# johannes-graeter/limo

Measured on NVIDIA H100. Metric: BA windows/s (30 KF, 3k LM, 40k obs), higher is better.
Workload: dtype f64

## Files before the change

limo_b200/csrc/kba_api.cu:

```cuda
#include <algorithm>
#include <atomic>
#include <chrono>
#include <cmath>
#include <cstdio>
#include <cstdlib>
#include <cstring>
#include <memory>
#include <string>
#include <thread>
#include <vector>

#include <cuda_runtime.h>

#include "kba_b200.h"
#include "kba_kernels.h"

using namespace kba;

static thread_local std::string g_last_error;
static int fail(int code, const std::string& msg) {
    g_last_error = msg;
    return code;
}
#define CU(call)                                                                                              \
// ... 713 lines not shown
        ws.free_rows = window_rows(w[i]);
        ws.n_chunks = d.n_chunks; ws.n_groups = d.n_groups; ws.n_lm = w[i].n_lm;
        d.nr_cap = nr_cap_of(ws.rows);
        d.plane_reg_weight = w[i].plane_reg_weight; d.plane_dist_fixed = w[i].plane_dist_fixed;
        d.s_off = soff;
        soff += (long long)d.nr_cap * d.nr_cap;
        kf += w[i].n_kf; cam += w[i].n_cam; lm += w[i].n_lm; obs += w[i].n_obs; chunks += d.n_chunks; gp += w[i].n_gp;
        bd.max_obs = std::max(bd.max_obs, w[i].n_obs); bd.max_lm = std::max(bd.max_lm, w[i].n_lm);
        bd.max_kf = std::max(bd.max_kf, w[i].n_kf); bd.max_gp = std::max(bd.max_gp, w[i].n_gp);
    }
    b->lc.knobs = read_knobs();
    b->lc.plan = make_plan(shapes.data(), n_windows, h->sm_count, b->lc.knobs, purpose);
    apply_plan(b);
    const int nr_cap_max = b->lc.plan.nr_cap_max;
    if (obs > 2000000000LL) { b->release(); delete b; return fail(KBA_ERR_CAPACITY, "batch exceeds 2^31 observations"); }
    if (nr_cap_max > kMaxReducedRows) {
        b->release();
        delete b;
        return fail(KBA_ERR_CAPACITY, "reduced system larger than 640 rows (106 keyframes, or 63 with ground-plane blocks)");
    }
    bd.tot_kf = kf; bd.tot_cam = cam; bd.tot_lm = lm; bd.tot_obs = obs; bd.tot_chunks = (int)chunks; bd.tot_gp = gp;
    bd.tot_groups = (int)groups;
    b->lc.sm_count = h->sm_count;
    bd.cost_parts = std::max((bd.max_obs + 255) / 256, (bd.max_obs / 16 + bd.max_lm / 32 + 4 + 7) / 8);
    bd.bs_parts = (bd.max_lm + 15) / 16;
    const bool hp = !b->lc.plan.device_pack;
    int bad = 0;
    bad |= b->desc.alloc(n_windows, true);
    bad |= b->pose0.alloc(7 * kf, true); bad |= b->plane0.alloc(4 * kf, true); bad |= b->kf_fixed.alloc(kf, true);
    bad |= b->cam.alloc(kCamStride * cam, true);
    bad |= b->lm0.alloc(3 * lm, hp); bad |= b->lm_weight.alloc(lm, hp); bad |= b->lm_ptr.alloc(lm + n_windows, hp);
    bad |= b->obs_kf.alloc(obs, hp); bad |= b->obs_cam.alloc(obs, hp); bad |= b->obs_lm.alloc(obs, hp);
    bad |= b->obs_u.alloc(obs, hp); bad |= b->obs_v.alloc(obs, hp); bad |= b->obs_d.alloc(obs, hp);
    bad |= b->kf_ptr.alloc(kf + n_windows, hp); bad |= b->pm_lm.alloc(obs, hp); bad |= b->pm_cam.alloc(obs, hp);
    bad |= b->pm_u.alloc(obs, hp); bad |= b->pm_v.alloc(obs, hp); bad |= b->pm_d.alloc(obs, hp);
    bad |= b->chunk_lm0.alloc(chunks, hp); bad |= b->chunk_lm1.alloc(chunks, hp);
    bad |= b->chunk_k0.alloc(chunks, hp); bad |= b->chunk_k1.alloc(chunks, hp);
    bad |= b->lm_orig.alloc(lm, hp); bad |= b->obs_rank.alloc(obs, hp);
    if (hp) bad |= b->obs_orig.alloc(obs, true);
    bad |= b->grp_k0.alloc(groups, hp); bad |= b->grp_k1.alloc(groups, hp);
    if (b->lc.plan.device_pack) {
        bad |= b->r_lm_ptr.alloc(lm + n_windows, true); bad |= b->r_obs_kf.alloc(obs, true); bad |= b->r_obs_cam.alloc(obs, true);
        bad |= b->r_obs_u.alloc(obs, true); bad |= b->r_obs_v.alloc(obs, true); bad |= b->r_obs_d.alloc(obs, true);
        bad |= b->r_lm_pos.alloc(3 * lm, true); bad |= b->r_lm_weight.alloc(lm, true); bad |= b->r_gp_lm.alloc(gp, true);
        bad |= b->lm_user.alloc(3 * lm, true); bad |= b->rej_user.alloc(lm, true);
        bad |= b->dev_alloc(&b->raw.lm_inv, lm);
    }
    bad |= b->dev_alloc(&bd.grp_t0, groups); bad |= b->dev_alloc(&bd.grp_t1, groups); bad |= b->dev_alloc(&bd.grp_rs, groups);
    bad |= b->dev_alloc(&bd.grp_tiles, groups);
    bad |= b->dev_alloc(&bd.lin_tile, (size_t)(obs / 16) + (size_t)(lm / 32) + 4 * (size_t)n_windows + 4);
#ifdef KBA_PROF
    bad |= b->dev_alloc(&bd.prof, 16);
    if (!bad) cudaMemset(bd.prof, 0, 16 * sizeof(unsigned long long));
#endif
    bad |= b->dev_alloc(&bd.rt[0], (size_t)kPoseStride * kf); bad |= b->dev_alloc(&bd.rt[1], (size_t)kPoseStride * kf);
    {
        bd.panel_cap = 0;
        bd.vpanel = nullptr;
        bad |= b->dev_alloc(&bd.chunk_poff, chunks); bad |= b->dev_alloc(&bd.chunk_rs, chunks);
    }
    bad |= b->dev_alloc(&bd.chunk_t0, chunks); bad |= b->dev_alloc(&bd.chunk_t1, chunks); bad |= b->dev_alloc(&bd.obs_row, obs);
    bad |= b->state.alloc(n_windows, true); bad |= b->log.alloc((size_t)n_windows * kIterLogCap, true);
    for (int q = 0; q < 2; ++q) { bad |= b->pose_out[q].alloc(7 * kf, true); bad |= b->lm_out[q].alloc(3 * lm, hp); }
    bad |= b->lm_active.alloc(lm, hp); bad |= b->n_active.alloc(1, true); bad |= b->jac_obs.alloc(1, true);
    bad |= b->plane_out[0].alloc(4 * kf, true); bad |= b->plane_out[1].alloc(4 * kf, true);
    bad |= b->gp_lm.alloc(gp, hp); bad |= b->gp_kf.alloc(gp, true); bad |= b->gp_weight.alloc(gp, true); bad |= b->gp_of_lm.alloc(lm, hp); bad |= b->gp_shared.alloc(gp, hp);
    bad |= b->dev_alloc(&bd.gp_lin, 14 * gp); bad |= b->dev_alloc(&bd.vgp, 30 * gp);
    bad |= b->dev_alloc(&bd.gp_kfb, gp ? 65 * (size_t)kf : 0);
    bad |= b->dev_alloc(&bd.gp_cost_x, n_windows); bad |= b->dev_alloc(&bd.gp_cost_c, n_windows);
    bad |= b->dev_alloc(&bd.off_pose, kf); bad |= b->dev_alloc(&bd.off_dir, kf); bad |= b->dev_alloc(&bd.off_dist, kf);
    bad |= b->dev_alloc(&bd.bkf, 27 * kf);
    bad |= b->dev_alloc(&bd.scale_f, (size_t)n_windows * nr_cap_max); bad |= b->dev_alloc(&bd.lambda_f, (size_t)n_windows * nr_cap_max);
    bad |= b->dev_alloc(&bd.grad_f, (size_t)n_windows * nr_cap_max); bad |= b->dev_alloc(&bd.delta_f, (size_t)n_windows * nr_cap_max);
    bad |= b->dev_alloc(&bd.lm_scale, 3 * lm); bad |= b->dev_alloc(&bd.lm_linv, 6 * lm); bad |= b->dev_alloc(&bd.lm_z, 3 * lm);
    bad |= b->dev_alloc(&bd.lm_g, 3 * lm); bad |= b->dev_alloc(&bd.lm_lambda, 3 * lm); bad |= b->dev_alloc(&bd.trim_val, 3 * lm);
    bad |= b->dev_alloc(&bd.trim_reject, lm);
    bad |= b->dev_alloc(&bd.res, 3 * obs); bad |= b->dev_alloc(&bd.jp, 18 * obs);
    if (!bd.fused) bad |= b->dev_alloc(&bd.jl, 9 * obs);
    else { bad |= b->dev_alloc(&bd.vobs, 18 * obs); bad |= b->dev_alloc(&bd.lm_run, lm); }
    bad |= b->dev_alloc(&bd.cost_part_x, (size_t)n_windows * bd.cost_parts); bad |= b->dev_alloc(&bd.cost_part_c, (size_t)n_windows * bd.cost_parts);
    bad |= b->dev_alloc(&bd.bs_part, (size_t)n_windows * bd.bs_parts * 4);
    bad |= b->dev_alloc(&bd.sred, (size_t)soff * bd.p_split); bad |= b->dev_alloc(&bd.amat, (size_t)soff);
    bad |= b->dev_alloc(&bd.chol_w, (size_t)n_windows * 32 * 32); bad |= b->dev_alloc(&bd.chol_invd, (size_t)n_windows * nr_cap_max);
    if (bad) {
        const std::string msg = std::string("device/pinned allocation failed: ") + cudaGetErrorString(cudaGetLastError());
        b->release(); delete b;
        return fail(KBA_ERR_CUDA, msg);
    }
    bd.desc = b->desc.d; bd.state = b->state.d; bd.log = b->log.d;
    bd.pose0 = b->pose0.d; bd.plane0 = b->plane0.d; bd.pose[0] = b->pose_out[0].d; bd.pose[1] = b->pose_out[1].d;
    bd.kf_fixed = b->kf_fixed.d; bd.cam = b->cam.d;
    bd.lm0 = b->lm0.d; bd.lm[0] = b->lm_out[0].d; bd.lm[1] = b->lm_out[1].d; bd.lm_weight = b->lm_weight.d;
    bd.lm_active = b->lm_active.d; bd.lm_ptr = b->lm_ptr.d;
    bd.obs_kf = b->obs_kf.d; bd.obs_cam = b->obs_cam.d; bd.obs_lm = b->obs_lm.d;
// ... 2106 lines not shown
```

limo_b200/csrc/kba_device.cuh:

```cuda
#pragma once
#include <cstdint>
#include <cuda_runtime.h>

#include "kba_plan.h"

namespace kba {

constexpr int kMaxKf = 128;
constexpr int kMaxCam = 8;
constexpr int kPoseStride = 12;
constexpr int kCamStride = 16;
constexpr int kIterLogCap = 160;

struct WinDesc {
    int n_kf, n_cam, n_lm, n_obs, n_gp;
    int kf_off, cam_off, lm_off, obs_off, gp_off;
    int chunk_off, n_chunks;
    int grp_off, n_groups;
    int scale_kf0, scale_kf1;
    double scale_weight, scale_value;
    double plane_reg_weight;
    int plane_dist_fixed, landmarks_fixed;
    int speed_kf;
    int idle;
// ... 42 lines not shown
    double radius, decrease_factor;
    double x_cost, x_norm, gmax;
    double f_model, f_step_sq, f_xnorm_sq, f_gmax;
    unsigned long long t_solve_start;
    SolveSummary solves[8];
};

struct BatchDev {
    int n_win;
    int max_obs, max_lm, max_kf, max_gp;
    long long tot_obs, tot_lm, tot_kf, tot_cam, tot_gp;
    WinDesc* desc;
    WinState* state;
    IterRecord* log;
    double* pose0;
    double* plane0;
    double* pose[2];
    double* rt[2];
    double* plane[2];
    uint8_t* kf_fixed;
    int* off_pose;
    int* off_dir;
    int* off_dist;
    double* bkf;
    double* scale_f;
    double* cam;
    double* lm0;
    double* lm[2];
    double* lm_weight;
    uint8_t* lm_active;
    uint8_t* lm_active0;
    int* lm_ptr;
    double* lm_scale;
    double* lm_linv;
    double* lm_z;
    double* lm_g;
    double* lm_lambda;
    double* trim_val;
    uint8_t* trim_reject;
    int* obs_kf;
    int* obs_cam;
    int* obs_lm;
    int* obs_rank;
    float* obs_u, *obs_v, *obs_d;
    int* kf_ptr;
    int* pm_lm;
    int* pm_cam;
// ... 337 lines not shown
```

limo_b200/csrc/kba_kernels.cu:

```cuda
#include "kba_device.cuh"
#include "kba_kernels.h"
#include "kba_regularisers.cuh"
#include "kba_controller.cuh"
#include "kba_prep.cuh"
#include "kba_linearize.cuh"

#include <cfloat>
#include <cstdio>
#include <cstdlib>
#include <cmath>
#include <type_traits>

namespace kba {

__global__ void __launch_bounds__(256) k_shard_planes(BatchDev bd) {
    if (bd.state[0].phase != PH_SOLVE_BEGIN) return;
    const WinDesc& wd = bd.desc[0];
    for (int k = threadIdx.x; k < wd.n_kf; k += blockDim.x) bd.kf_gp_glob[k] = 0;
    __syncthreads();
    for (int j = threadIdx.x; j < bd.lm_total; j += blockDim.x) {
        const int kp = (int)bd.gp_kf_glob[j];
        if (kp > 0 && bd.act_glob[j]) bd.kf_gp_glob[kp - 1] = 1;
    }
}
// ... 154 lines not shown
                const int t0 = bd.chunk_t0[wd.chunk_off + c], t1 = bd.chunk_t1[wd.chunk_off + c];
                int rs = 0;
                if (t1 > t0) {
                    const int rows = 8 * (t1 - t0) + ((trhs >= t0 && trhs < t1) ? 0 : 8);
                    rs = ((rows - 4 + 15) / 16) * 16 + 4;
                }
                bd.chunk_rs[wd.chunk_off + c] = rs;
                bd.chunk_poff[wd.chunk_off + c] = poff;
                poff += 96 * rs;
            }
        }
    }
}

__global__ void __launch_bounds__(256) k_panel_zero(BatchDev bd) {
    const int w = blockIdx.y;
    if (bd.fused || bd.state[w].phase != PH_SOLVE_BEGIN || bd.desc[w].landmarks_fixed) return;
    double2* p = reinterpret_cast<double2*>(bd.vpanel + bd.desc[w].panel_off);
    const long long n2 = bd.panel_cap / 2;
    for (long long i = (long long)blockIdx.x * blockDim.x + threadIdx.x; i < n2; i += (long long)gridDim.x * blockDim.x)
        p[i] = make_double2(0.0, 0.0);
}

template <bool kJac, int kMinBlocks, typename TLin, bool kJl = true>
__global__ void __launch_bounds__(256, kMinBlocks) k_eval_obs(BatchDev bd, SolveParams sp, int tiles) {
    const int w = blockIdx.y;
    WinState& st = bd.state[w];
    const WinDesc& wd = bd.desc[w];
    const int n_obs = wd.n_obs, obs_off = wd.obs_off, lm_off = wd.lm_off;
    if (st.phase != PH_ITERATE) return;
    if (kJac && !st.need_linearize) return;
    if (!kJac && st.solve_failed) return;
    __shared__ __align__(16) double s_pose[kMaxKf * kPoseStride];
    __shared__ __align__(16) double s_cam[kMaxCam * kCamStride];
    __shared__ __align__(8) uint64_t s_bar;
    __shared__ double s_red[8];
    __shared__ int s_cnt[8];
    constexpr bool kF32 = sizeof(TLin) == 4;
    __shared__ float s_pose_f[kF32 ? kMaxKf * kPoseStride : 1];
    __shared__ float s_cam_f[kF32 ? kMaxCam * kCamStride : 1];
    const int buf = kJac ? st.cur : 1 - st.cur;
    const double* __restrict__ lm_buf = bd.lm[buf];
    const int i0 = blockIdx.x * tiles * 256 + threadIdx.x;
    int idx_b = (i0 < n_obs) ? bd.obs_lm[(size_t)obs_off + i0] : -1;
    int idx_a = (tiles > 1 && i0 + 256 < n_obs) ? bd.obs_lm[(size_t)obs_off + i0 + 256] : -1;
    int L = -1, kfi = 0, cami = 0, row = -1;
    float u = 0.f, v = 0.f, d = 0.f;
    double p0 = 0, p1 = 0, p2 = 0, wgt = 0;
    unsigned char act = 0;
    if (idx_b >= 0) {
        const size_t o = (size_t)obs_off + i0;
        L = lm_off + idx_b;
        kfi = bd.obs_kf[o]; cami = bd.obs_cam[o];
        if (kJac) row = bd.obs_row[o];
        u = bd.obs_u[o]; v = bd.obs_v[o]; d = bd.obs_d[o];
        p0 = lm_buf[3 * (size_t)L]; p1 = lm_buf[3 * (size_t)L + 1]; p2 = lm_buf[3 * (size_t)L + 2];
        wgt = bd.lm_weight[L];
        act = bd.lm_active[L];
    }
    stage_window_bulk(wd, bd.rt[buf], bd.cam, s_pose, s_cam, &s_bar);
    if (kF32) {
        for (int i = threadIdx.x; i < wd.n_kf * kPoseStride; i += blockDim.x) s_pose_f[i] = (float)s_pose[i];
        for (int i = threadIdx.x; i < wd.n_cam * kCamStride; i += blockDim.x) s_cam_f[i] = (float)s_cam[i];
        __syncthreads();
    }
    double cost = 0.0;
    int done = 0;
#pragma unroll 1
    for (int t = 0; t < tiles; ++t) {
        const int i_n = i0 + (t + 1) * 256;
        int Ln = -1, kfn = 0, camn = 0, rown = -1;
        float un = 0.f, vn = 0.f, dn = 0.f;
        double q0 = 0, q1 = 0, q2 = 0, wn = 0;
        unsigned char actn = 0;
        if (idx_a >= 0) {
            const size_t o = (size_t)obs_off + i_n;
            Ln = lm_off + idx_a;
            kfn = bd.obs_kf[o]; camn = bd.obs_cam[o];
            if (kJac) rown = bd.obs_row[o];
            un = bd.obs_u[o]; vn = bd.obs_v[o]; dn = bd.obs_d[o];
            q0 = lm_buf[3 * (size_t)Ln]; q1 = lm_buf[3 * (size_t)Ln + 1]; q2 = lm_buf[3 * (size_t)Ln + 2];
            wn = bd.lm_weight[Ln];
            actn = bd.lm_active[Ln];
        }
        idx_a = (t + 2 < tiles && i_n + 256 < n_obs) ? bd.obs_lm[(size_t)obs_off + i_n + 256] : -1;
        if (L >= 0 && act) {
            const size_t o = (size_t)obs_off + i0 + t * 256;
            const int k = kfi, c = cami;
            const double p[3] = {p0, p1, p2};
            double hr = 0.0;
            bool ok;
            if (kJac && kF32) {
                double r[3], raw[2];
                ok = eval_observation<double, false>(
                    s_pose + kPoseStride * k, s_cam + kCamStride * c, p, (double)u, (double)v, (double)d, wgt,
                    sp.reprojection_thres * sp.reprojection_thres, sp.depth_thres * sp.depth_thres, r, nullptr, nullptr, hr,
                    raw);
                if (ok) {
                    const float pf[3] = {(float)p0, (float)p1, (float)p2};
                    float hrf;
                    float* resf = reinterpret_cast<float*>(bd.res) + o;
                    float* jpf = reinterpret_cast<float*>(bd.jp) + o;
                    float* jlf = reinterpret_cast<float*>(bd.jl) + o;
                    eval_observation_store<float, kJl>(
                        s_pose_f + kPoseStride * k, s_cam_f + kCamStride * c, pf, u, v, d, (float)wgt,
                        (float)(sp.reprojection_thres * sp.reprojection_thres), (float)(sp.depth_thres * sp.depth_thres),
                        resf, jpf, jlf, (size_t)bd.tot_obs, row >= 0 || !kJl, hrf);
                }
            } else if (kJac) {
                ok = eval_observation_store<double, kJl>(
                    s_pose + kPoseStride * k, s_cam + kCamStride * c, p, (double)u, (double)v, (double)d, wgt,
                    sp.reprojection_thres * sp.reprojection_thres, sp.depth_thres * sp.depth_thres, bd.res + o, bd.jp + o,
                    bd.jl + o, (size_t)bd.tot_obs, row >= 0 || !kJl, hr);
            } else {
                double r[3], raw[2];
                ok = eval_observation<double, false>(
                    s_pose + kPoseStride * k, s_cam + kCamStride * c, p, (double)u, (double)v, (double)d, wgt,
                    sp.reprojection_thres * sp.reprojection_thres, sp.depth_thres * sp.depth_thres, r, nullptr, nullptr,
                    hr, raw);
            }
            if (!ok) {
                st.eval_failed = 1;
            } else {
                cost += hr;
                ++done;
            }
        }
        L = Ln; kfi = kfn; cami = camn; row = rown; u = un; v = vn; d = dn; p0 = q0; p1 = q1; p2 = q2; wgt = wn; act = actn;
    }
    cost = warp_sum(cost);
    if (kJac) done = __reduce_add_sync(0xffffffffu, done);
    if ((threadIdx.x & 31) == 0) { s_red[threadIdx.x >> 5] = cost; s_cnt[threadIdx.x >> 5] = done; }
    __syncthreads();
    if (threadIdx.x < tiles) {
        double s = 0.0;
        if (threadIdx.x == 0)
            for (int q = 0; q < 8; ++q) s += s_red[q];
        const int slot = blockIdx.x * tiles + threadIdx.x;
        if (slot < bd.cost_parts) (kJac ? bd.cost_part_x : bd.cost_part_c)[(size_t)w * bd.cost_parts + slot] = s;
    }
    if (kJac && threadIdx.x == 0) {
        int cnt = 0;
        for (int q = 0; q < 8; ++q) cnt += s_cnt[q];
        if (cnt) atomicAdd(bd.jac_obs, (unsigned long long)cnt);
    }
}

constexpr int kEvalTiles = 8;
template <bool kJac>
static void launch_eval_obs(const BatchDev& bd, const SolveParams& sp, cudaStream_t s) {
    const dim3 g((bd.max_obs + 256 * kEvalTiles - 1) / (256 * kEvalTiles), bd.n_win);
    if (!kJac) { k_eval_obs<false, 4, double><<<g, 256, 0, s>>>(bd, sp, kEvalTiles); return; }
    if (bd.precision == 1) {
        if (bd.fused) k_eval_obs<true, 2, float, false><<<g, 256, 0, s>>>(bd, sp, kEvalTiles);
        else k_eval_obs<true, 2, float, true><<<g, 256, 0, s>>>(bd, sp, kEvalTiles);
    } else {
        if (bd.fused) k_eval_obs<true, 2, double, false><<<g, 256, 0, s>>>(bd, sp, kEvalTiles);
        else k_eval_obs<true, 2, double, true><<<g, 256, 0, s>>>(bd, sp, kEvalTiles);
    }
    LCHK("k_eval_obs");
}

template <bool kJac>
__global__ void __launch_bounds__(256) k_gp_eval(BatchDev bd, SolveParams sp) {
    const int w = blockIdx.x;
    const WinState& st = bd.state[w];
    if (st.phase != PH_ITERATE) return;
    if (kJac && !st.need_linearize) return;
    if (!kJac && st.solve_failed) return;
    const WinDesc& wd = bd.desc[w];
    if (wd.n_gp == 0) return;
    __shared__ double s_red[8];
    const int buf = kJac ? st.cur : 1 - st.cur;
    const size_t TG = (size_t)bd.tot_gp;
    double cost = 0.0;
    for (int gi = threadIdx.x; gi < wd.n_gp; gi += blockDim.x) {
        const size_t G = (size_t)wd.gp_off + gi;
        const int L = wd.lm_off + bd.gp_lm[G];
        if (!bd.lm_active[L]) continue;
        const int k = bd.gp_kf[G];
        const double* ps = bd.pose[buf] + 7 * (size_t)(wd.kf_off + k);
// ... 57 lines not shown
        const int e = lane + 32 * s;
        int a = 0, b = 0;
        if (e < 55) { while ((a + 1) * (a + 2) / 2 <= e) ++a; b = e - a * (a + 1) / 2; }
        else if (e < 65) { a = e - 55; b = -1; }
        else { a = -1; b = -1; }
        ea[s] = a; eb[s] = b;
    }
    for (int gi = 0; gi < wd.n_gp; ++gi) {
        const size_t G = (size_t)wd.gp_off + gi;
        if (bd.gp_kf[G] != k || !bd.lm_active[wd.lm_off + bd.gp_lm[G]]) continue;
#pragma unroll
        for (int s = 0; s < 3; ++s) {
            if (ea[s] < 0) continue;
            const double va = bd.gp_lin[(1 + ea[s]) * TG + G];
            const double vb = (eb[s] >= 0) ? bd.gp_lin[(1 + eb[s]) * TG + G] : bd.gp_lin[G];
            acc[s] += va * vb;
        }
    }
#pragma unroll
    for (int s = 0; s < 3; ++s)
        if (ea[s] >= 0) bd.gp_kfb[(size_t)(wd.kf_off + k) * 65 + lane + 32 * s] = acc[s];
}

__global__ void __launch_bounds__(256, 2) k_pose_hessian(BatchDev bd, SolveParams sp) {
    const int w = blockIdx.y, k = blockIdx.x;
    const WinState& st = bd.state[w];
    if (st.phase != PH_ITERATE || !st.need_linearize) return;
    const WinDesc& wd = bd.desc[w];
    if (k >= wd.n_kf || bd.off_pose[wd.kf_off + k] < 0) return;
    __shared__ double s_pose[kPoseStride];
    __shared__ double s_cam[kMaxCam * kCamStride];
    __shared__ double s_red[8][27];
    __shared__ double s_acc[9][256];
    __shared__ long long s_ob;
    __shared__ int s_lm_off, s_e1;
    if (threadIdx.x == 0) {
        s_ob = wd.obs_off; s_lm_off = wd.lm_off; s_e1 = bd.kf_ptr[wd.kf_off + w + k + 1];
        const double* p = bd.pose[st.cur] + 7 * (size_t)(wd.kf_off + k);
        double R[9];
        quat_to_rot<double>(p, R);
        for (int i = 0; i < 9; ++i) s_pose[i] = R[i];
        s_pose[9] = p[4]; s_pose[10] = p[5]; s_pose[11] = p[6];
    }
    for (int i = threadIdx.x; i < wd.n_cam * kCamStride; i += blockDim.x) s_cam[i] = bd.cam[(size_t)wd.cam_off * kCamStride + i];
    __syncthreads();
    double acc[18];
#pragma unroll
    for (int q = 0; q < 18; ++q) acc[q] = 0.0;
#pragma unroll
    for (int q = 0; q < 9; ++q) s_acc[q][threadIdx.x] = 0.0;
    const int* kp = bd.kf_ptr + wd.kf_off + w;
    const int e0 = kp[k], e1 = kp[k + 1];
    const double* __restrict__ lm_buf = bd.lm[st.cur];
    const size_t ob = (size_t)wd.obs_off;
    int e = e0 + threadIdx.x;
    int idx_b = (e < e1) ? bd.pm_lm[ob + e] : -1;
    int idx_a = (e + (int)blockDim.x < e1) ? bd.pm_lm[ob + e + blockDim.x] : -1;
    int L = -1, cam = 0;
    float u = 0.f, v = 0.f, d = 0.f;
    double p0 = 0, p1 = 0, p2 = 0, wgt = 0;
    unsigned char act = 0;
    if (idx_b >= 0) {
        L = wd.lm_off + idx_b;
        cam = bd.pm_cam[ob + e]; u = bd.pm_u[ob + e]; v = bd.pm_v[ob + e]; d = bd.pm_d[ob + e];
        p0 = lm_buf[3 * (size_t)L]; p1 = lm_buf[3 * (size_t)L + 1]; p2 = lm_buf[3 * (size_t)L + 2];
        wgt = bd.lm_weight[L]; act = bd.lm_active[L];
    }
#pragma unroll 1
    for (; e < s_e1; e += blockDim.x) {
        asm volatile("" ::: "memory");
        const size_t obs0 = (size_t)s_ob;
        const int e_end = s_e1, lm0 = s_lm_off;
        const int en = e + blockDim.x;
        int Ln = -1, camn = 0;
        float un = 0.f, vn = 0.f, dn = 0.f;
        double q0 = 0, q1 = 0, q2 = 0, wn = 0;
        unsigned char actn = 0;
        if (idx_a >= 0) {
            Ln = lm0 + idx_a;
            camn = bd.pm_cam[obs0 + en]; un = bd.pm_u[obs0 + en]; vn = bd.pm_v[obs0 + en]; dn = bd.pm_d[obs0 + en];
            q0 = lm_buf[3 * (size_t)Ln]; q1 = lm_buf[3 * (size_t)Ln + 1]; q2 = lm_buf[3 * (size_t)Ln + 2];
            wn = bd.lm_weight[Ln]; actn = bd.lm_active[Ln];
        }
        idx_a = (en + (int)blockDim.x < e_end) ? bd.pm_lm[obs0 + en + blockDim.x] : -1;
        if (act) {
            const double p[3] = {p0, p1, p2};
            double r[3], m[9], a[3], raw[2], hr;
            if (eval_factored<double, true, false>(s_pose, s_cam + kCamStride * cam, p, (double)u, (double)v, (double)d,
                                                   wgt, sp.reprojection_thres * sp.reprojection_thres,
                                                   sp.depth_thres * sp.depth_thres, r, m, a, hr, raw)) {
                double mm[6], h[3];
                gram_factored(m, mm);
#pragma unroll
                for (int c = 0; c < 3; ++c) h[c] = m[c] * r[0] + m[3 + c] * r[1] + m[6 + c] * r[2];
#pragma unroll
                for (int i = 0; i < 3; ++i) {
                    const int i1 = (i + 1) % 3, i2 = (i + 2) % 3;
                    double pr[3];
#pragma unroll
                    for (int c = 0; c < 3; ++c) pr[c] = 2.0 * (a[i1] * mm[sym3(i2, c)] - a[i2] * mm[sym3(i1, c)]);
                    const int qd = 6 * i - i * (i - 1) / 2;
#pragma unroll
                    for (int j = i; j < 3; ++j) {
                        const int j1 = (j + 1) % 3, j2 = (j + 2) % 3;
                        acc[qd + j - i] += 2.0 * (a[j1] * pr[j2] - a[j2] * pr[j1]);
                    }
#pragma unroll
                    for (int c = 0; c < 3; ++c) acc[qd + 3 - i + c] += pr[c];
                    acc[15 + i] += 2.0 * (a[i1] * h[i2] - a[i2] * h[i1]);
                }
#pragma unroll
                for (int q = 0; q < 6; ++q) s_acc[q][threadIdx.x] += mm[q];
#pragma unroll
                for (int c = 0; c < 3; ++c) s_acc[6 + c][threadIdx.x] += h[c];
            }
        }
        L = Ln; cam = camn; u = un; v = vn; d = dn; p0 = q0; p1 = q1; p2 = q2; wgt = wn; act = actn;
    }
#pragma unroll
    for (int q = 0; q < 27; ++q) {
        const double t = q < 15 ? acc[q] : q < 21 ? s_acc[q - 15][threadIdx.x] : q < 24 ? acc[q - 6] : s_acc[q - 18][threadIdx.x];
        const double v = warp_sum(t);
        if ((threadIdx.x & 31) == 0) s_red[threadIdx.x >> 5][q] = v;
    }
    __syncthreads();
    if (threadIdx.x < 27) {
        double s = 0.0;
        for (int q = 0; q < 8; ++q) s += s_red[q][threadIdx.x];
        bd.bkf[(size_t)(wd.kf_off + k) * 27 + threadIdx.x] = s;
    }
}

constexpr int kLC = 32;
constexpr int kKC = 3 * kLC;

__device__ __forceinline__ int gp_row(const BatchDev& bd, const WinDesc& wd, int k, int r) {
    if (r < 6) { const int o = bd.off_pose[wd.kf_off + k]; return o < 0 ? -1 : o + r; }
    if (r < 9) { const int o = bd.off_dir[wd.kf_off + k]; return o < 0 ? -1 : o + r - 6; }
    return bd.off_dist[wd.kf_off + k];
}

__device__ __forceinline__ void dmma(double& c0, double& c1, double a, double b) {
    asm volatile("mma.sync.aligned.m8n8k4.row.col.f64.f64.f64.f64 {%0,%1}, {%2}, {%3}, {%0,%1};\n"
                 : "+d"(c0), "+d"(c1)
                 : "d"(a), "d"(b));
}

constexpr int kGS = 64 + 4;

__global__ void __launch_bounds__(256, 2) k_schur_syrk(BatchDev bd) {
    const int w = blockIdx.z;
    const WinState& st = bd.state[w];
// ... 405 lines not shown
            int rr[8], cc[8];
#pragma unroll
            for (int u = 0; u < 8; ++u) {
                const int idx = idx0 + u * nth;
                const int r = idx / ld, c = idx - r * ld;
                const bool skip = idx >= total || (kTiled ? (c >= rows || (c >> 3) > (r >> 3)) : (c > r || c >= n + 1));
                rr[u] = skip ? -1 : r; cc[u] = c;
                double s = 0.0;
                if (!skip && !wd.landmarks_fixed && c <= r && r <= n && !(r == n && c == n))
                    for (int p = 0; p < np; ++p) s += sp0[p * pstride + (size_t)r * ld + c];
                v[u] = s;
            }
#pragma unroll
            for (int u = 0; u < 8; ++u)
                if (rr[u] >= 0) A(rr[u], cc[u]) = -v[u];
        }
    }
    __syncthreads();
    PHASE_MARK(1);
    for (int idx = tid; idx < wd.n_kf * 27; idx += nth) {
        const int k = idx / 27, q = idx - 27 * k;
        const int off = bd.off_pose[wd.kf_off + k];
        if (off < 0) continue;
        const double v = bd.bkf[(size_t)(wd.kf_off + k) * 27 + q];
        if (q < 21) {
            int a = 0, rem = q;
            while (rem >= 6 - a) { rem -= 6 - a; ++a; }
            const int b = a + rem;
            A(off + b, off + a) += v;
            if (a == b) s_fdiag[off + a] = v;
        } else {
            s_g[off + q - 21] = v;
        }
    }
    __syncthreads();
    if (wd.n_gp > 0 || bd.shard_gp) {
        for (int idx = tid; idx < wd.n_kf * 65; idx += nth) {
            const int k = idx / 65, e = idx - 65 * k;
            int a, b;
            if (e < 55) { a = 0; while ((a + 1) * (a + 2) / 2 <= e) ++a; b = e - a * (a + 1) / 2; }
            else { a = e - 55; b = -1; }
            const int ra = gp_row(bd, wd, k, a);
            if (ra < 0) continue;
            const double v = bd.gp_kfb[(size_t)(wd.kf_off + k) * 65 + e];
            if (b < 0) { s_g[ra] += v; continue; }
            const int rb = gp_row(bd, wd, k, b);
            if (rb < 0) continue;
// ... 632 lines not shown
            const double* p = bd.bs_part + (size_t)q * 4;
            a += p[0]; b += p[1]; c += p[2]; g = fmax(g, p[3]);
        }
        for (int q = lane; q < bd.cost_parts; q += 32) cc += bd.cost_part_c[q];
    }
    a = warp_sum(a); b = warp_sum(b); c = warp_sum(c); g = warp_max(g);
    cc = warp_sum(cc);
    if (lane == 0) {
        bd.xs[0] = a; bd.xs[1] = b; bd.xs[2] = c; bd.xs[3] = cc;
        bd.xs[4] = (st.phase == PH_ITERATE && st.eval_failed) ? 1.0 : 0.0;
        bd.xs[5] = (st.phase == PH_ITERATE && wd.n_gp > 0) ? bd.gp_cost_c[0] : 0.0;
        for (int r = 0; r < bd.shard_world; ++r) bd.xs[16 + r] = (r == bd.shard_rank) ? g : 0.0;
    }
}
__host__ __device__ inline long long shard_gp_doubles(int shard_gp, int n_kf) { return shard_gp ? 65LL * n_kf + 1 : 0; }
__global__ void __launch_bounds__(256) k_shard_pack(BatchDev bd) {
    const WinState& st = bd.state[0];
    const WinDesc& wd = bd.desc[0];
    const size_t n_s = (size_t)wd.nr_cap * wd.nr_cap, n_b = (size_t)wd.n_kf * 27, n_c = (size_t)bd.shard_cost_parts;
    const size_t n_g = (size_t)shard_gp_doubles(bd.shard_gp, wd.n_kf), n_kb = (size_t)wd.n_kf * 65;
    const size_t i = (size_t)blockIdx.x * blockDim.x + threadIdx.x;
    const bool on = st.phase == PH_ITERATE, gp = on && wd.n_gp > 0;
    if (i < n_s) bd.x_send[i] = on ? bd.sred[i] : 0.0;
    else if (i < n_s + n_b) bd.x_send[i] = on ? bd.bkf[i - n_s] : 0.0;
    else if (i < n_s + n_b + n_kb && n_g) bd.x_send[i] = gp ? bd.gp_kfb[i - n_s - n_b] : 0.0;
    else if (i == n_s + n_b + n_kb && n_g) bd.x_send[i] = gp ? bd.gp_cost_x[0] : 0.0;
    else if (i < n_s + n_b + n_g + n_c) {
        const size_t q = i - n_s - n_b - n_g;
        bd.x_send[i] = (on && q < (size_t)bd.cost_parts) ? bd.cost_part_x[q] : 0.0;
    }
    else if (i == n_s + n_b + n_g + n_c) bd.x_send[i] = (on && st.eval_failed) ? 1.0 : 0.0;
    else if (i == n_s + n_b + n_g + n_c + 1) bd.x_send[i] = (on && st.solve_failed) ? 1.0 : 0.0;
}
__global__ void k_shard_flags(BatchDev bd) {
    WinState& st = bd.state[0];
    if (threadIdx.x != 0 || st.phase != PH_ITERATE) return;
    const WinDesc& wd = bd.desc[0];
    const double* f = bd.x_recv + (size_t)wd.nr_cap * wd.nr_cap + (size_t)wd.n_kf * 27 + shard_gp_doubles(bd.shard_gp, wd.n_kf) +
                      bd.shard_cost_parts;
    if (f[0] > 0.0) st.eval_failed = 1;
    if (f[1] > 0.0 && !st.solve_failed) st.solve_failed = 1;
}
__global__ void __launch_bounds__(256) k_shard_trim_scatter(BatchDev bd) {
    const WinState& st = bd.state[0];
    if (st.phase != PH_TRIM) return;
    const WinDesc& wd = bd.desc[0];
    const int j = blockIdx.x * blockDim.x + threadIdx.x;
// ... 260 lines not shown
    const int B = bd.n_win;
    const dim3 g_obs((bd.max_obs + 255) / 256, B);
    const dim3 g_lm((bd.max_lm + 63) / 64, B);
    if (!bd.fused) k_panel_zero<<<dim3(64, B), 256, 0, s>>>(bd);
    LCHK("k_panel_zero");
    if (bd.sharded && bd.shard_gp) k_shard_planes<<<1, 256, 0, s>>>(bd);
    LCHK("k_shard_planes");
    k_solve_begin<<<B, kBeginThreads, 0, s>>>(bd, sp); LCHK("k_solve_begin");
    const bool timed = lc.time_jacobian && lc.ev_pool && *lc.ev_used + 2 <= lc.ev_cap;
    const bool lin1 = bd.lin1 != 0;
    if (lin1) {
        if (bd.tot_gp > 0) {
            k_gp_eval<true><<<B, 256, 0, s>>>(bd, sp);
            k_gp_blocks<<<dim3((bd.max_kf + 7) / 8, B), 256, 0, s>>>(bd);
        }
        LCHK("k_gp_eval");
        if (timed) cudaEventRecord(lc.ev_pool[(*lc.ev_used)++], s);
        const int n_units = (lin_tile_bound(bd.max_obs, bd.max_lm) + kLinWarps - 1) / kLinWarps;
        const dim3 g_lin(strided_grid(lc.knobs.lin_grid, n_units, 1, 8, B, lc.sm_count, kLinMinBlocks, 6), B);
        if ((int)g_lin.x < n_units) k_linearize<true><<<g_lin, kLinThreads, 0, s>>>(bd, sp, n_units);
        else k_linearize<false><<<g_lin, kLinThreads, 0, s>>>(bd, sp, n_units);
        LCHK("k_linearize");
        if (timed) cudaEventRecord(lc.ev_pool[(*lc.ev_used)++], s);
        k_pose_hessian<<<dim3(bd.max_kf, B), 256, 0, s>>>(bd, sp); LCHK("k_pose_hessian");
    } else {
        if (timed) cudaEventRecord(lc.ev_pool[(*lc.ev_used)++], s);
        launch_eval_obs<true>(bd, sp, s);
        if (timed) cudaEventRecord(lc.ev_pool[(*lc.ev_used)++], s);
        if (bd.tot_gp > 0) {
            k_gp_eval<true><<<B, 256, 0, s>>>(bd, sp);
            k_gp_blocks<<<dim3((bd.max_kf + 7) / 8, B), 256, 0, s>>>(bd);
        }
        LCHK("k_gp_eval");
        k_pose_hessian<<<dim3(bd.max_kf, B), 256, 0, s>>>(bd, sp); LCHK("k_pose_hessian");
    }
    if (bd.fused) {
        if (!lin1) {
            k_landmark_reduce<true><<<dim3((bd.max_lm + 15) / 16, B), 256, 0, s>>>(bd, sp); LCHK("k_landmark_reduce");
            k_obs_v2<<<g_obs, 256, 0, s>>>(bd); LCHK("k_obs_v2");
        }
        const dim3 gf(bd.p_split, B);
        if (lc.plan.fused_slots == 7) k_schur_fused<7><<<gf, 512, schur_fused_smem(), s>>>(bd);
        else k_schur_fused<6><<<gf, 512, schur_fused_smem(), s>>>(bd);
        LCHK("k_schur_fused");
    } else {
        k_landmark_reduce<false><<<dim3((bd.max_lm + 15) / 16, B), 256, 0, s>>>(bd, sp); LCHK("k_landmark_reduce");
        for (int round = 0; round <= lc.max_rank; ++round) k_obs_v<<<g_obs, 256, 0, s>>>(bd, round);
        LCHK("k_obs_v");
        if (bd.tot_gp > 0) k_gp_panel<<<dim3((bd.max_gp * 10 + 255) / 256, B), 256, 0, s>>>(bd);
        LCHK("k_gp_panel");
    }
    if (bd.fused) {
    } else if (lc.plan.small_syrk) {
        k_schur_syrk_tma<<<dim3(bd.p_split, B), 512, schur_tma_smem(), s>>>(bd); LCHK("k_schur_syrk_tma");
    } else {
        const int nb = lc.plan.nr_cap_max / 64;
        k_schur_syrk<<<dim3(nb * (nb + 1) / 2, bd.p_split, B), 256, schur_smem(), s>>>(bd); LCHK("k_schur_syrk");
    }
    const dim3 g_red((lc.plan.nr_cap_max * lc.plan.nr_cap_max + 255) / 256, B);
    BatchDev bc = bd;
    if (bd.sharded) {
        if (bd.p_split > 1) k_sred_reduce<<<g_red, 256, 0, s>>>(bd, 1);
        LCHK("k_sred_reduce");
        const LaunchCfg::WinDescHost& wh = lc.shard_win;
        const long long n_s = (long long)wh.nr_cap * wh.nr_cap, n_b = (long long)wh.n_kf * 27, n_g = shard_gp_doubles(bd.shard_gp, wh.n_kf);
        const long long n_x = n_s + n_b + n_g + bd.shard_cost_parts + 2;
        k_shard_pack<<<(unsigned)((n_x + 255) / 256), 256, 0, s>>>(bd); LCHK("k_shard_pack");
        if (int rc = lc.xchg.allreduce(lc.xchg.user, bd.x_send, bd.x_recv, n_x, 0, s)) return rc;
        k_shard_flags<<<1, 32, 0, s>>>(bd); LCHK("k_shard_flags");
        bc.sred = bd.x_recv; bc.bkf = bd.x_recv + n_s; bc.cost_part_x = bd.x_recv + n_s + n_b + n_g; bc.cost_parts = bd.shard_cost_parts;
        if (n_g) { bc.gp_kfb = bd.x_recv + n_s + n_b; bc.gp_cost_x = bd.x_recv + n_s + n_b + 65LL * wh.n_kf; }
        k_sred_reduce<<<g_red, 256, 0, s>>>(bc, 2); LCHK("k_sred_reduce");
    } else if (bd.p_split > 1) {
        k_sred_reduce<<<g_red, 256, 0, s>>>(bd, 0); LCHK("k_sred_reduce");
    }
    if (bd.solve_tiled) {
        k_reduced_solve<true><<<B, 512, solve_tiled_smem(lc.plan.nr_cap_max), s>>>(bc, sp, 0); LCHK("k_reduced_solve");
    } else if (!bd.solve_split) {
        k_reduced_solve<false><<<B, 512, solve_smem(lc.plan.nr_cap_max), s>>>(bc, sp, 0); LCHK("k_reduced_solve");
    } else {
        k_reduced_solve<false><<<B, 512, solve_smem(lc.plan.nr_cap_max), s>>>(bc, sp, 1); LCHK("k_reduced_solve");
        const int strips = (lc.plan.nr_cap_max + 7) / 8;
        for (int kb = 0; kb < lc.plan.nr_cap_max; kb += kNB) {
            k_chol_diag<<<B, 32, 0, s>>>(bc, kb); LCHK("k_chol_diag");
            k_chol_panel<<<dim3((strips + 15) / 16, B), 512, 0, s>>>(bc, kb); LCHK("k_chol_panel");
            k_chol_trail<<<dim3(bd.solve_split, B), 512, trail_smem(lc.plan.nr_cap_max), s>>>(bc, kb); LCHK("k_chol_trail");
        }
        k_reduced_solve<false><<<B, 512, solve_smem(lc.plan.nr_cap_max), s>>>(bc, sp, 2); LCHK("k_reduced_solve");
    }
    if (bd.fused) {
        const int n_units = (bd.max_lm + 15) / 16;
        const int gx = strided_grid(lc.knobs.bs_grid, n_units, 1, 3, B, lc.sm_count, 2, 8);
        if (gx < n_units) k_backsub_v<true><<<dim3(gx, B), 256, 0, s>>>(bd, n_units);
        else k_backsub_v<false><<<dim3(n_units, B), 256, 0, s>>>(bd, n_units);
    }
    else k_backsub<<<dim3((bd.max_lm + 15) / 16, B), 256, 0, s>>>(bd);
    LCHK("k_backsub");
    launch_eval_obs<false>(bd, sp, s);
    if (bd.tot_gp > 0) k_gp_eval<false><<<B, 256, 0, s>>>(bd, sp);
    LCHK("k_gp_eval");
    if (bd.sharded) {
        k_shard_scalars<<<1, 32, 0, s>>>(bd); LCHK("k_shard_scalars");
        if (int rc = lc.xchg.allreduce(lc.xchg.user, bd.xs, bd.xs, 16 + bd.shard_world, 0, s)) return rc;
    }
    k_lm_update<<<(B * 32 + 127) / 128, 128, 0, s>>>(bd, sp); LCHK("k_lm_update");
    k_trim_eval<<<g_lm, 256, 0, s>>>(bd, sp); LCHK("k_trim_eval");
    if (bd.sharded) {
        k_shard_trim_scatter<<<(bd.max_lm + 255) / 256, 256, 0, s>>>(bd); LCHK("k_shard_trim_scatter");
        if (int rc = lc.xchg.allreduce(lc.xchg.user, bd.trim_send, bd.trim_glob, 3LL * bd.lm_total, 0, s)) return rc;
    }
    k_trim_select<<<B, 512, 0, s>>>(bd, sp); LCHK("k_trim_select");
    if (cnt) {
        const int gp = bd.tot_gp > 0 ? 1 : 0;
        const int prep = lin1 ? 1 : 2 + (bd.fused ? 1 : lc.max_rank + 1 + gp);
        cnt->launches_total += gp; cnt->launches_prep += gp;
        if (bd.sharded && bd.shard_gp) cnt->launches_total += 1;
        const int split = (!bd.solve_tiled && bd.solve_split) ? 1 + 3 * ((lc.plan.nr_cap_max + kNB - 1) / kNB) : 0;
        cnt->launches_total += (bd.fused ? 0 : 1) + 1 + 1 + gp + prep + 1 + (bd.p_split > 1 ? 1 : 0) + 1 + split + 1 + 1 + gp + 1 + 2;
        cnt->launches_jacobian += 1; cnt->launches_prep += prep + gp; cnt->launches_schur += 1; cnt->launches_solve += 2;
        cnt->launches_backsub += 1; cnt->launches_cost += 1 + gp; cnt->launches_update += 1; cnt->launches_trim += 2;
    }
// ... 8 lines not shown
__global__ void __launch_bounds__(256) k_loop_cond(BatchDev bd, cudaGraphConditionalHandle handle, int* pass, int max_passes) {
    int active = 0;
    for (int w = threadIdx.x; w < bd.n_win; w += blockDim.x) active += (bd.state[w].phase != PH_DONE) ? 1 : 0;
    active = __syncthreads_count(active > 0);
    if (threadIdx.x == 0) {
        const int p = *pass + 1;
        *pass = p;
        *bd.n_active = active;
        cudaGraphSetConditional(handle, (active > 0 && p < max_passes) ? 1u : 0u);
    }
}
void launch_loop_cond(const BatchDev& bd, unsigned long long handle, int* pass, int max_passes, cudaStream_t s) {
    k_loop_cond<<<1, 256, 0, s>>>(bd, (cudaGraphConditionalHandle)handle, pass, max_passes);
}

__global__ void k_force_linearize(BatchDev bd) {
    const int w = blockIdx.x * blockDim.x + threadIdx.x;
    if (w >= bd.n_win) return;
    WinState& st = bd.state[w];
    st.phase = PH_ITERATE; st.need_linearize = 1; st.iter0 = 1; st.cur = 0; st.eval_failed = 0; st.solve_failed = 0;
}
void launch_jacobian_only(const BatchDev& bd, const SolveParams& sp, cudaStream_t s) {
    const dim3 g_obs((bd.max_obs + 255) / 256, bd.n_win);
    launch_eval_obs<true>(bd, sp, s);
}
template <typename TLin>
__global__ void k_expand_jl(BatchDev bd, double* out) {
    const WinDesc& wd = bd.desc[0];
    const int i = blockIdx.x * blockDim.x + threadIdx.x;
    if (i >= wd.n_obs) return;
    const size_t o = (size_t)wd.obs_off + i, T = (size_t)bd.tot_obs;
    const double* R = bd.rt[0] + kPoseStride * (size_t)(wd.kf_off + bd.obs_kf[o]);
    const TLin* jp = reinterpret_cast<const TLin*>(bd.jp);
    for (int r = 0; r < 3; ++r) {
        const double m0 = (double)jp[(6 * r + 3) * T + o], m1 = (double)jp[(6 * r + 4) * T + o], m2 = (double)jp[(6 * r + 5) * T + o];
        for (int c = 0; c < 3; ++c) out[(size_t)(3 * r + c) * T + o] = m0 * R[c] + m1 * R[3 + c] + m2 * R[6 + c];
    }
}
void launch_expand_jl(const BatchDev& bd, double* out, cudaStream_t s) {
    const int n = (int)bd.tot_obs;
    if (bd.precision) k_expand_jl<float><<<(n + 255) / 256, 256, 0, s>>>(bd, out);
    else k_expand_jl<double><<<(n + 255) / 256, 256, 0, s>>>(bd, out);
    LCHK("k_expand_jl");
}
void launch_force_linearize(const BatchDev& bd, cudaStream_t s) {
    k_solve_begin<<<bd.n_win, kBeginThreads, 0, s>>>(bd, SolveParams{}); LCHK("k_solve_begin");
    k_force_linearize<<<(bd.n_win + 127) / 128, 128, 0, s>>>(bd); LCHK("k_force_linearize");
// ... 4 lines not shown
```

Measured before the change: 1454.

## Fuse candidate cost evaluation into pose Hessian kernel and double-buffer bkf

Replaces the separate candidate-cost eval_obs pass after backsubstitution with a k_pose_hessian<true> launch. That launch evaluates the candidate state, accumulates cost per keyframe and also precomputes the pose Hessian blocks into a second bkf buffer. The intent is that an accepted step can reuse these blocks, so the next linearization skips k_pose_hessian unless iter0. This removes a redundant per-observation pass, at the cost of a heavier candidate kernel that builds the Hessian even for steps that get rejected. It also adds buffer-index bookkeeping across cur flips.

```diff
diff --git a/limo_b200/csrc/kba_api.cu b/limo_b200/csrc/kba_api.cu
--- a/limo_b200/csrc/kba_api.cu
+++ b/limo_b200/csrc/kba_api.cu
@@ -759,7 +759,7 @@
     bd.tot_kf = kf; bd.tot_cam = cam; bd.tot_lm = lm; bd.tot_obs = obs; bd.tot_chunks = (int)chunks; bd.tot_gp = gp;
     bd.tot_groups = (int)groups;
     b->lc.sm_count = h->sm_count;
-    bd.cost_parts = std::max((bd.max_obs + 255) / 256, (bd.max_obs / 16 + bd.max_lm / 32 + 4 + 7) / 8);
+    bd.cost_parts = std::max(std::max((bd.max_obs + 255) / 256, (bd.max_obs / 16 + bd.max_lm / 32 + 4 + 7) / 8), bd.max_kf);
     bd.bs_parts = (bd.max_lm + 15) / 16;
     const bool hp = !b->lc.plan.device_pack;
     int bad = 0;
@@ -806,7 +806,7 @@
     bad |= b->dev_alloc(&bd.gp_kfb, gp ? 65 * (size_t)kf : 0);
     bad |= b->dev_alloc(&bd.gp_cost_x, n_windows); bad |= b->dev_alloc(&bd.gp_cost_c, n_windows);
     bad |= b->dev_alloc(&bd.off_pose, kf); bad |= b->dev_alloc(&bd.off_dir, kf); bad |= b->dev_alloc(&bd.off_dist, kf);
-    bad |= b->dev_alloc(&bd.bkf, 27 * kf);
+    bad |= b->dev_alloc(&bd.bkf[0], 27 * kf); bad |= b->dev_alloc(&bd.bkf[1], 27 * kf);
     bad |= b->dev_alloc(&bd.scale_f, (size_t)n_windows * nr_cap_max); bad |= b->dev_alloc(&bd.lambda_f, (size_t)n_windows * nr_cap_max);
     bad |= b->dev_alloc(&bd.grad_f, (size_t)n_windows * nr_cap_max); bad |= b->dev_alloc(&bd.delta_f, (size_t)n_windows * nr_cap_max);
     bad |= b->dev_alloc(&bd.lm_scale, 3 * lm); bad |= b->dev_alloc(&bd.lm_linv, 6 * lm); bad |= b->dev_alloc(&bd.lm_z, 3 * lm);
diff --git a/limo_b200/csrc/kba_device.cuh b/limo_b200/csrc/kba_device.cuh
--- a/limo_b200/csrc/kba_device.cuh
+++ b/limo_b200/csrc/kba_device.cuh
@@ -88,7 +88,7 @@
     int* off_pose;
     int* off_dir;
     int* off_dist;
-    double* bkf;
+    double* bkf[2];
     double* scale_f;
     double* cam;
     double* lm0;
diff --git a/limo_b200/csrc/kba_kernels.cu b/limo_b200/csrc/kba_kernels.cu
--- a/limo_b200/csrc/kba_kernels.cu
+++ b/limo_b200/csrc/kba_kernels.cu
@@ -200,15 +200,13 @@
         p[i] = make_double2(0.0, 0.0);
 }
 
-template <bool kJac, int kMinBlocks, typename TLin, bool kJl = true>
+template <int kMinBlocks, typename TLin, bool kJl = true>
 __global__ void __launch_bounds__(256, kMinBlocks) k_eval_obs(BatchDev bd, SolveParams sp, int tiles) {
     const int w = blockIdx.y;
     WinState& st = bd.state[w];
     const WinDesc& wd = bd.desc[w];
     const int n_obs = wd.n_obs, obs_off = wd.obs_off, lm_off = wd.lm_off;
-    if (st.phase != PH_ITERATE) return;
-    if (kJac && !st.need_linearize) return;
-    if (!kJac && st.solve_failed) return;
+    if (st.phase != PH_ITERATE || !st.need_linearize) return;
     __shared__ __align__(16) double s_pose[kMaxKf * kPoseStride];
     __shared__ __align__(16) double s_cam[kMaxCam * kCamStride];
     __shared__ __align__(8) uint64_t s_bar;
@@ -217,7 +215,7 @@
     constexpr bool kF32 = sizeof(TLin) == 4;
     __shared__ float s_pose_f[kF32 ? kMaxKf * kPoseStride : 1];
     __shared__ float s_cam_f[kF32 ? kMaxCam * kCamStride : 1];
-    const int buf = kJac ? st.cur : 1 - st.cur;
+    const int buf = st.cur;
     const double* __restrict__ lm_buf = bd.lm[buf];
     const int i0 = blockIdx.x * tiles * 256 + threadIdx.x;
     int idx_b = (i0 < n_obs) ? bd.obs_lm[(size_t)obs_off + i0] : -1;
@@ -230,7 +228,7 @@
         const size_t o = (size_t)obs_off + i0;
         L = lm_off + idx_b;
         kfi = bd.obs_kf[o]; cami = bd.obs_cam[o];
-        if (kJac) row = bd.obs_row[o];
+        row = bd.obs_row[o];
         u = bd.obs_u[o]; v = bd.obs_v[o]; d = bd.obs_d[o];
         p0 = lm_buf[3 * (size_t)L]; p1 = lm_buf[3 * (size_t)L + 1]; p2 = lm_buf[3 * (size_t)L + 2];
         wgt = bd.lm_weight[L];
@@ -255,7 +253,7 @@
             const size_t o = (size_t)obs_off + i_n;
             Ln = lm_off + idx_a;
             kfn = bd.obs_kf[o]; camn = bd.obs_cam[o];
-            if (kJac) rown = bd.obs_row[o];
+            rown = bd.obs_row[o];
             un = bd.obs_u[o]; vn = bd.obs_v[o]; dn = bd.obs_d[o];
             q0 = lm_buf[3 * (size_t)Ln]; q1 = lm_buf[3 * (size_t)Ln + 1]; q2 = lm_buf[3 * (size_t)Ln + 2];
             wn = bd.lm_weight[Ln];
@@ -268,7 +266,7 @@
             const double p[3] = {p0, p1, p2};
             double hr = 0.0;
             bool ok;
-            if (kJac && kF32) {
+            if (kF32) {
                 double r[3], raw[2];
                 ok = eval_observation<double, false>(
                     s_pose + kPoseStride * k, s_cam + kCamStride * c, p, (double)u, (double)v, (double)d, wgt,
@@ -285,17 +283,11 @@
                         (float)(sp.reprojection_thres * sp.reprojection_thres), (float)(sp.depth_thres * sp.depth_thres),
                         resf, jpf, jlf, (size_t)bd.tot_obs, row >= 0 || !kJl, hrf);
                 }
-            } else if (kJac) {
+            } else {
                 ok = eval_observation_store<double, kJl>(
                     s_pose + kPoseStride * k, s_cam + kCamStride * c, p, (double)u, (double)v, (double)d, wgt,
                     sp.reprojection_thres * sp.reprojection_thres, sp.depth_thres * sp.depth_thres, bd.res + o, bd.jp + o,
                     bd.jl + o, (size_t)bd.tot_obs, row >= 0 || !kJl, hr);
-            } else {
-                double r[3], raw[2];
-                ok = eval_observation<double, false>(
-                    s_pose + kPoseStride * k, s_cam + kCamStride * c, p, (double)u, (double)v, (double)d, wgt,
-                    sp.reprojection_thres * sp.reprojection_thres, sp.depth_thres * sp.depth_thres, r, nullptr, nullptr,
-                    hr, raw);
             }
             if (!ok) {
                 st.eval_failed = 1;
@@ -307,7 +299,7 @@
         L = Ln; kfi = kfn; cami = camn; row = rown; u = un; v = vn; d = dn; p0 = q0; p1 = q1; p2 = q2; wgt = wn; act = actn;
     }
     cost = warp_sum(cost);
-    if (kJac) done = __reduce_add_sync(0xffffffffu, done);
+    done = __reduce_add_sync(0xffffffffu, done);
     if ((threadIdx.x & 31) == 0) { s_red[threadIdx.x >> 5] = cost; s_cnt[threadIdx.x >> 5] = done; }
     __syncthreads();
     if (threadIdx.x < tiles) {
@@ -315,9 +307,9 @@
         if (threadIdx.x == 0)
             for (int q = 0; q < 8; ++q) s += s_red[q];
         const int slot = blockIdx.x * tiles + threadIdx.x;
-        if (slot < bd.cost_parts) (kJac ? bd.cost_part_x : bd.cost_part_c)[(size_t)w * bd.cost_parts + slot] = s;
-    }
-    if (kJac && threadIdx.x == 0) {
+        if (slot < bd.cost_parts) bd.cost_part_x[(size_t)w * bd.cost_parts + slot] = s;
+    }
+    if (threadIdx.x == 0) {
         int cnt = 0;
         for (int q = 0; q < 8; ++q) cnt += s_cnt[q];
         if (cnt) atomicAdd(bd.jac_obs, (unsigned long long)cnt);
@@ -325,16 +317,14 @@
 }
 
 constexpr int kEvalTiles = 8;
-template <bool kJac>
 static void launch_eval_obs(const BatchDev& bd, const SolveParams& sp, cudaStream_t s) {
     const dim3 g((bd.max_obs + 256 * kEvalTiles - 1) / (256 * kEvalTiles), bd.n_win);
-    if (!kJac) { k_eval_obs<false, 4, double><<<g, 256, 0, s>>>(bd, sp, kEvalTiles); return; }
     if (bd.precision == 1) {
-        if (bd.fused) k_eval_obs<true, 2, float, false><<<g, 256, 0, s>>>(bd, sp, kEvalTiles);
-        else k_eval_obs<true, 2, float, true><<<g, 256, 0, s>>>(bd, sp, kEvalTiles);
+        if (bd.fused) k_eval_obs<2, float, false><<<g, 256, 0, s>>>(bd, sp, kEvalTiles);
+        else k_eval_obs<2, float, true><<<g, 256, 0, s>>>(bd, sp, kEvalTiles);
     } else {
-        if (bd.fused) k_eval_obs<true, 2, double, false><<<g, 256, 0, s>>>(bd, sp, kEvalTiles);
-        else k_eval_obs<true, 2, double, true><<<g, 256, 0, s>>>(bd, sp, kEvalTiles);
+        if (bd.fused) k_eval_obs<2, double, false><<<g, 256, 0, s>>>(bd, sp, kEvalTiles);
+        else k_eval_obs<2, double, true><<<g, 256, 0, s>>>(bd, sp, kEvalTiles);
     }
     LCHK("k_eval_obs");
 }
@@ -438,21 +428,28 @@
         if (ea[s] >= 0) bd.gp_kfb[(size_t)(wd.kf_off + k) * 65 + lane + 32 * s] = acc[s];
 }
 
+template <bool kCand>
 __global__ void __launch_bounds__(256, 2) k_pose_hessian(BatchDev bd, SolveParams sp) {
     const int w = blockIdx.y, k = blockIdx.x;
-    const WinState& st = bd.state[w];
-    if (st.phase != PH_ITERATE || !st.need_linearize) return;
+    WinState& st = bd.state[w];
+    if (st.phase != PH_ITERATE) return;
+    if (kCand ? st.solve_failed != 0 : !(st.need_linearize && st.iter0)) return;
     const WinDesc& wd = bd.desc[w];
-    if (k >= wd.n_kf || bd.off_pose[wd.kf_off + k] < 0) return;
+    if (kCand && k >= wd.n_kf) {
+        if (threadIdx.x == 0) bd.cost_part_c[(size_t)w * bd.cost_parts + k] = 0.0;
+        return;
+    }
+    if (k >= wd.n_kf || (!kCand && bd.off_pose[wd.kf_off + k] < 0)) return;
+    const int buf = kCand ? 1 - st.cur : st.cur;
     __shared__ double s_pose[kPoseStride];
     __shared__ double s_cam[kMaxCam * kCamStride];
-    __shared__ double s_red[8][27];
-    __shared__ double s_acc[9][256];
+    __shared__ double s_red[8][kCand ? 28 : 27];
+    __shared__ double s_acc[kCand ? 10 : 9][256];
     __shared__ long long s_ob;
     __shared__ int s_lm_off, s_e1;
     if (threadIdx.x == 0) {
         s_ob = wd.obs_off; s_lm_off = wd.lm_off; s_e1 = bd.kf_ptr[wd.kf_off + w + k + 1];
-        const double* p = bd.pose[st.cur] + 7 * (size_t)(wd.kf_off + k);
+        const double* p = bd.pose[buf] + 7 * (size_t)(wd.kf_off + k);
         double R[9];
         quat_to_rot<double>(p, R);
         for (int i = 0; i < 9; ++i) s_pose[i] = R[i];
@@ -464,10 +461,10 @@
 #pragma unroll
     for (int q = 0; q < 18; ++q) acc[q] = 0.0;
 #pragma unroll
-    for (int q = 0; q < 9; ++q) s_acc[q][threadIdx.x] = 0.0;
+    for (int q = 0; q < (kCand ? 10 : 9); ++q) s_acc[q][threadIdx.x] = 0.0;
     const int* kp = bd.kf_ptr + wd.kf_off + w;
     const int e0 = kp[k], e1 = kp[k + 1];
-    const double* __restrict__ lm_buf = bd.lm[st.cur];
+    const double* __restrict__ lm_buf = bd.lm[buf];
     const size_t ob = (size_t)wd.obs_off;
     int e = e0 + threadIdx.x;
     int idx_b = (e < e1) ? bd.pm_lm[ob + e] : -1;
@@ -502,9 +499,10 @@
         if (act) {
             const double p[3] = {p0, p1, p2};
             double r[3], m[9], a[3], raw[2], hr;
-            if (eval_factored<double, true, false>(s_pose, s_cam + kCamStride * cam, p, (double)u, (double)v, (double)d,
+            if (eval_factored<double, true, kCand>(s_pose, s_cam + kCamStride * cam, p, (double)u, (double)v, (double)d,
                                                    wgt, sp.reprojection_thres * sp.reprojection_thres,
                                                    sp.depth_thres * sp.depth_thres, r, m, a, hr, raw)) {
+                if (kCand) s_acc[9][threadIdx.x] += hr;
                 double mm[6], h[3];
                 gram_factored(m, mm);
 #pragma unroll
@@ -529,21 +527,25 @@
                 for (int q = 0; q < 6; ++q) s_acc[q][threadIdx.x] += mm[q];
 #pragma unroll
                 for (int c = 0; c < 3; ++c) s_acc[6 + c][threadIdx.x] += h[c];
+            } else if (kCand) {
+                bd.state[blockIdx.y].eval_failed = 1;
             }
         }
         L = Ln; cam = camn; u = un; v = vn; d = dn; p0 = q0; p1 = q1; p2 = q2; wgt = wn; act = actn;
     }
 #pragma unroll
-    for (int q = 0; q < 27; ++q) {
+    for (int q = 0; q < (kCand ? 28 : 27); ++q) {
         const double t = q < 15 ? acc[q] : q < 21 ? s_acc[q - 15][threadIdx.x] : q < 24 ? acc[q - 6] : s_acc[q - 18][threadIdx.x];
         const double v = warp_sum(t);
         if ((threadIdx.x & 31) == 0) s_red[threadIdx.x >> 5][q] = v;
     }
     __syncthreads();
-    if (threadIdx.x < 27) {
+    if (threadIdx.x < (kCand ? 28 : 27)) {
         double s = 0.0;
         for (int q = 0; q < 8; ++q) s += s_red[q][threadIdx.x];
-        bd.bkf[(size_t)(wd.kf_off + k) * 27 + threadIdx.x] = s;
+        const int half = kCand ? 1 - ((const volatile WinState&)st).cur : ((const volatile WinState&)st).cur;
+        if (threadIdx.x == 27) bd.cost_part_c[(size_t)w * bd.cost_parts + k] = s;
+        else if (bd.off_pose[wd.kf_off + k] >= 0) bd.bkf[half][(size_t)(wd.kf_off + k) * 27 + threadIdx.x] = s;
     }
 }
 
@@ -995,7 +997,7 @@
         const int k = idx / 27, q = idx - 27 * k;
         const int off = bd.off_pose[wd.kf_off + k];
         if (off < 0) continue;
-        const double v = bd.bkf[(size_t)(wd.kf_off + k) * 27 + q];
+        const double v = bd.bkf[st.cur][(size_t)(wd.kf_off + k) * 27 + q];
         if (q < 21) {
             int a = 0, rem = q;
             while (rem >= 6 - a) { rem -= 6 - a; ++a; }
@@ -1674,7 +1676,7 @@
     const size_t i = (size_t)blockIdx.x * blockDim.x + threadIdx.x;
     const bool on = st.phase == PH_ITERATE, gp = on && wd.n_gp > 0;
     if (i < n_s) bd.x_send[i] = on ? bd.sred[i] : 0.0;
-    else if (i < n_s + n_b) bd.x_send[i] = on ? bd.bkf[i - n_s] : 0.0;
+    else if (i < n_s + n_b) bd.x_send[i] = on ? bd.bkf[st.cur][i - n_s] : 0.0;
     else if (i < n_s + n_b + n_kb && n_g) bd.x_send[i] = gp ? bd.gp_kfb[i - n_s - n_b] : 0.0;
     else if (i == n_s + n_b + n_kb && n_g) bd.x_send[i] = gp ? bd.gp_cost_x[0] : 0.0;
     else if (i < n_s + n_b + n_g + n_c) {
@@ -1981,17 +1983,17 @@
         else k_linearize<false><<<g_lin, kLinThreads, 0, s>>>(bd, sp, n_units);
         LCHK("k_linearize");
         if (timed) cudaEventRecord(lc.ev_pool[(*lc.ev_used)++], s);
-        k_pose_hessian<<<dim3(bd.max_kf, B), 256, 0, s>>>(bd, sp); LCHK("k_pose_hessian");
+        k_pose_hessian<false><<<dim3(bd.max_kf, B), 256, 0, s>>>(bd, sp); LCHK("k_pose_hessian");
     } else {
         if (timed) cudaEventRecord(lc.ev_pool[(*lc.ev_used)++], s);
-        launch_eval_obs<true>(bd, sp, s);
+        launch_eval_obs(bd, sp, s);
         if (timed) cudaEventRecord(lc.ev_pool[(*lc.ev_used)++], s);
         if (bd.tot_gp > 0) {
             k_gp_eval<true><<<B, 256, 0, s>>>(bd, sp);
             k_gp_blocks<<<dim3((bd.max_kf + 7) / 8, B), 256, 0, s>>>(bd);
         }
         LCHK("k_gp_eval");
-        k_pose_hessian<<<dim3(bd.max_kf, B), 256, 0, s>>>(bd, sp); LCHK("k_pose_hessian");
+        k_pose_hessian<false><<<dim3(bd.max_kf, B), 256, 0, s>>>(bd, sp); LCHK("k_pose_hessian");
     }
     if (bd.fused) {
         if (!lin1) {
@@ -2027,7 +2029,7 @@
         k_shard_pack<<<(unsigned)((n_x + 255) / 256), 256, 0, s>>>(bd); LCHK("k_shard_pack");
         if (int rc = lc.xchg.allreduce(lc.xchg.user, bd.x_send, bd.x_recv, n_x, 0, s)) return rc;
         k_shard_flags<<<1, 32, 0, s>>>(bd); LCHK("k_shard_flags");
-        bc.sred = bd.x_recv; bc.bkf = bd.x_recv + n_s; bc.cost_part_x = bd.x_recv + n_s + n_b + n_g; bc.cost_parts = bd.shard_cost_parts;
+        bc.sred = bd.x_recv; bc.bkf[0] = bc.bkf[1] = bd.x_recv + n_s; bc.cost_part_x = bd.x_recv + n_s + n_b + n_g; bc.cost_parts = bd.shard_cost_parts;
         if (n_g) { bc.gp_kfb = bd.x_recv + n_s + n_b; bc.gp_cost_x = bd.x_recv + n_s + n_b + 65LL * wh.n_kf; }
         k_sred_reduce<<<g_red, 256, 0, s>>>(bc, 2); LCHK("k_sred_reduce");
     } else if (bd.p_split > 1) {
@@ -2055,7 +2057,7 @@
     }
     else k_backsub<<<dim3((bd.max_lm + 15) / 16, B), 256, 0, s>>>(bd);
     LCHK("k_backsub");
-    launch_eval_obs<false>(bd, sp, s);
+    k_pose_hessian<true><<<dim3(bd.max_kf, B), 256, 0, s>>>(bd, sp); LCHK("k_pose_hessian");
     if (bd.tot_gp > 0) k_gp_eval<false><<<B, 256, 0, s>>>(bd, sp);
     LCHK("k_gp_eval");
     if (bd.sharded) {
@@ -2110,7 +2112,7 @@
 }
 void launch_jacobian_only(const BatchDev& bd, const SolveParams& sp, cudaStream_t s) {
     const dim3 g_obs((bd.max_obs + 255) / 256, bd.n_win);
-    launch_eval_obs<true>(bd, sp, s);
+    launch_eval_obs(bd, sp, s);
 }
 template <typename TLin>
 __global__ void k_expand_jl(BatchDev bd, double* out) {
```

Result: faster. 1483, median of 6 (+2.0%).
